# AvishaiBarnoy/membrane_solver

Measured on AMD Instinct MI355X. Metric: minimizer steps/sec (energy+grad+CG) on 2M-facet icosphere, higher is better.
Workload: dtype f64

## Files before the change

### include/membrane_hip.h

```cpp
#ifndef MEMBRANE_HIP_H
#define MEMBRANE_HIP_H

#include <stddef.h>
#include <stdint.h>

#ifdef __cplusplus
extern "C" {
#endif

#define MS_OK 0
#define MS_ERR_INVALID (-1)
#define MS_ERR_HIP (-2)
#define MS_ERR_TILE_CAPACITY (-3)
#define MS_ERR_STATE (-4)
#define MS_ERR_NOMEM (-5)

#define MS_MOD_SURFACE 1u
#define MS_MOD_BENDING 2u
#define MS_MOD_VOLUME_PENALTY 4u
#define MS_CON_VOLUME 8u
#define MS_TRACK_VOLUME 16u
#define MS_MOD_TILT 32u
#define MS_MOD_BENDING_TILT 64u
#define MS_MOD_TILT_SMOOTH 128u
// ... 275 lines not shown
                  double tol, ms_step_result *out);
int64_t ms_shard_exchange_count(const ms_ctx *ctx);
int ms_shard_chain_stats(const ms_ctx *ctx, int64_t stats[8]);
int ms_shard_comm_ranks(ms_ctx *ctx);
int ms_shard_peer_memory_kind(const ms_ctx *ctx);

size_t ms_state_bytes(const ms_ctx *ctx);
int ms_rebind_state(ms_ctx *ctx, void *device_base, size_t bytes);

int ms_device_buffer(ms_ctx *ctx, int buffer, void **dev_ptr, size_t *bytes);
int ms_shard_info(ms_ctx *ctx, int64_t *nvp, int64_t *row0, int64_t *row1,
                  int64_t *rows_per_shard);
int ms_tile_stats(ms_ctx *ctx, int64_t *n_tiles, int64_t *facet_instances,
                  int64_t *max_halo, int64_t *lds_bytes_energy,
                  int64_t *lds_bytes_gradient);

#define MS_PROF_KINDS 13
int ms_profile_enable(ms_ctx *ctx, int on);
int ms_profile_read(ms_ctx *ctx, double total_ms[MS_PROF_KINDS],
                    int64_t launches[MS_PROF_KINDS]);

int ms_queue_stats(ms_ctx *ctx, int64_t stats[8]);
int ms_direction_stats(ms_ctx *ctx, int64_t *skipped, int64_t *materialized);
int ms_exec_stats(ms_ctx *ctx, int64_t stats[4]);
int ms_resident_stats(ms_ctx *ctx, int64_t stats[4]);

#define MS_PIN_STAGE_FIXED 0
#define MS_PIN_STAGE_PLANE_GROUP 1
#define MS_PIN_STAGE_CIRCLE_GROUP 2
#define MS_PIN_OP_PLANE 0
// ... 44 lines not shown
```

### membrane_solver_amd/_lib.py

```python

from __future__ import annotations

import ctypes
import os
import subprocess

_PKG = os.path.dirname(os.path.abspath(__file__))
LIB_PATH = os.environ.get("MEMBRANE_HIP_LIB") or os.path.join(_PKG, "libmembrane_hip.so")
_CSRC = os.path.join(_PKG, "csrc")

MS_OK = 0
MS_ERR = {-1: "MS_ERR_INVALID", -2: "MS_ERR_HIP", -3: "MS_ERR_TILE_CAPACITY",
          -4: "MS_ERR_STATE", -5: "MS_ERR_NOMEM"}

MS_MOD_SURFACE = 1
MS_MOD_BENDING = 2
MS_MOD_VOLUME_PENALTY = 4
MS_CON_VOLUME = 8
MS_TRACK_VOLUME = 16
MS_MOD_TILT = 32
MS_MOD_BENDING_TILT = 64
MS_MOD_TILT_SMOOTH = 128
MS_MOD_TILT_IN, MS_MOD_TILT_OUT, MS_MOD_TILT_SMOOTH_IN, MS_MOD_TILT_SMOOTH_OUT = 256, 512, 1024, 2048
MS_MOD_BENDING_TILT_IN, MS_MOD_BENDING_TILT_OUT = 4096, 8192
# ... 167 lines not shown
    "ms_shard_set_allgather": (ctypes.c_int, [_P, ALLGATHER_FN, _P]),
    "ms_shard_step": (ctypes.c_int, [_P, ctypes.POINTER(ms_stepper_params), ctypes.c_double, ctypes.c_double,
                                     ctypes.POINTER(ms_step_result)]),
    "ms_shard_exchange_count": (ctypes.c_int64, [_P]),
    "ms_shard_chain_stats": (ctypes.c_int, [_P, _I64]),
    "ms_shard_comm_ranks": (ctypes.c_int, [_P]),
    "ms_shard_peer_memory_kind": (ctypes.c_int, [_P]),
    "ms_state_bytes": (ctypes.c_size_t, [_P]),
    "ms_rebind_state": (ctypes.c_int, [_P, _P, ctypes.c_size_t]),
    "ms_fetch_scalars": (ctypes.c_int, [_P, _D]),
    "ms_store_scalars": (ctypes.c_int, [_P, _D]),
    "ms_device_buffer": (ctypes.c_int, [_P, ctypes.c_int, ctypes.POINTER(_P),
                                        ctypes.POINTER(ctypes.c_size_t)]),
    "ms_shard_info": (ctypes.c_int, [_P, _I64, _I64, _I64, _I64]),
    "ms_tile_stats": (ctypes.c_int, [_P, _I64, _I64, _I64, _I64, _I64]),
    "ms_profile_enable": (ctypes.c_int, [_P, ctypes.c_int]),
    "ms_profile_read": (ctypes.c_int, [_P, _D, _I64]),
    "ms_queue_stats": (ctypes.c_int, [_P, _I64]),
    "ms_direction_stats": (ctypes.c_int, [_P, _I64, _I64]),
    "ms_exec_stats": (ctypes.c_int, [_P, _I64]),
    "ms_resident_stats": (ctypes.c_int, [_P, _I64]),
    "ms_set_pins": (ctypes.c_int, [_P, ctypes.c_int, _D, ctypes.c_int, _I32, _I32, _I32, _I32, _I32, ctypes.c_int,
                                   ctypes.c_int, _I32, _I32, _I32, ctypes.c_int, _I32, _I32, _I32]),
    "ms_enforce_pins": (ctypes.c_int, [_P]),
    "ms_pin_stats": (ctypes.c_int, [_P, _I64]),
    "ms_tsearch_stats": (ctypes.c_int, [_P, _I64]),
    "ms_exec_trace": (ctypes.c_int, [_P, ctypes.c_int, _D, ctypes.c_int, ctypes.POINTER(ctypes.c_int)]),
    "ms_shard_peer_export": (ctypes.c_int, [_P, _P]),
    "ms_shard_peer_open": (ctypes.c_int, [_P, _P]),
    "ms_shard_peer_local": (ctypes.c_int, [_P, ctypes.POINTER(_P), ctypes.POINTER(_P)]),
# ... 92 lines not shown
```

### membrane_solver_amd/csrc/ms_api_context.inc

```
extern "C" {

const char* ms_version(void) { return "membrane_hip 0.1 (gfx950)"; }

int ms_device_count(void) {
  int n = 0;
  hipError_t e = hipGetDeviceCount(&n);
  if (e != hipSuccess) {
    g_last_error = std::string("hipGetDeviceCount: ") + hipGetErrorString(e);
    return MS_ERR_HIP;
  }
  return n;
}

const char* ms_last_error(const ms_ctx* ctx) {
  return ctx ? ctx->err.c_str() : g_last_error.c_str();
}

int ms_create(ms_ctx** out, int device, int nv, int nf, const double* positions,
              const int32_t* tri, const uint8_t* fixed, const uint8_t* boundary,
              const uint8_t* body_facets, int tile_vertices, int shard_rank, int shard_count) {
  if (!out) return fail(nullptr, MS_ERR_INVALID, "ms_create: out is NULL");
  *out = nullptr;
  if (shard_count < 1 || shard_rank < 0 || shard_rank >= shard_count)
    return fail(nullptr, MS_ERR_INVALID, "ms_create: bad shard_rank/shard_count");
// ... 43 lines not shown
  CREATE_HIP(hipSetDevice(device));
  CREATE_HIP(hipStreamCreateWithFlags(&c->stream, hipStreamNonBlocking));
  c->own_stream = true;
  CREATE_CHK(upload(c, &c->d_perm, t.perm));
  CREATE_CHK(upload(c, &c->d_tile_facet_off, t.tile_facet_off));
  CREATE_CHK(upload(c, &c->d_tile_facets, t.tile_facets));
  if (t.own + t.max_halo <= 1024) {
    std::vector<uint32_t> packed(t.tile_facets.size());
    for (size_t i = 0; i < packed.size(); ++i) {
      const TileFacet& f = t.tile_facets[i];
      packed[i] = (uint32_t)f.l0 | ((uint32_t)f.l1 << 10) | ((uint32_t)f.l2 << 20) | ((uint32_t)(f.flags & 3u) << 30);
    }
    CREATE_CHK(upload(c, &c->d_tile_facets32, packed));
  }
  CREATE_CHK(upload(c, &c->d_tile_halo_off, t.tile_halo_off));
  CREATE_CHK(upload(c, &c->d_halo_ids, t.halo_ids));
  CREATE_CHK(upload(c, &c->d_tile_ent_off, t.tile_ent_off));
  CREATE_CHK(upload(c, &c->d_tile_voff, t.tile_voff));
  CREATE_CHK(upload(c, &c->d_vent, t.vent));
  {
    std::vector<double> ones(t.tile_facets.size(), 1.0);
    CREATE_CHK(upload(c, &c->d_tf_gamma, ones));
  }
  {
    std::vector<uint8_t> fl((size_t)t.nvp, VF_FIXED);
    for (int i = 0; i < nv; ++i) {
      const int e = t.perm[i];
      uint8_t f = 0;
      if (fixed && fixed[e]) f |= VF_FIXED;
      if (boundary && boundary[e]) {
// ... 128 lines not shown
            g_host_timing.n, g_host_timing.sum_gap / g_host_timing.n, g_host_timing.max_gap,
            g_host_timing.sum_launch / g_host_timing.n);
    g_host_timing.n = 0;
    g_host_timing.sum_gap = g_host_timing.sum_launch = g_host_timing.max_gap = 0.0;
  }
  if (!c) return;
  (void)hipSetDevice(c->device);
  if (c->exec_on) {
    (void)c->exec.flush();
    exec_detach(&c->exec);
    c->exec_on = false;
  }
  if (c->stream) (void)hipStreamSynchronize(c->stream);
  if (!c->own_state) c->state = nullptr;
  void* ptrs[] = {c->d_perm, c->d_tile_facet_off, c->d_tile_facets, c->d_tile_facets32, c->d_tf_gamma, c->d_volgrad_cache,
                  c->d_tile_halo_off, c->d_halo_ids, c->d_tile_ent_off, c->d_tile_voff, c->d_vent,
                  c->d_vflags, c->d_kappa, c->d_c0, c->tf[0].tilts, c->tf[0].grad, c->tf[0].trial, c->d_bt_vert, c->d_tn, c->tf[0].dir, c->tf[0].minv,
                  c->tf[1].tilts, c->tf[1].grad, c->tf[1].trial, c->tf[1].dir, c->tf[1].minv,
                  c->tf[2].tilts, c->tf[2].grad, c->tf[2].trial, c->tf[2].dir, c->tf[2].minv,
                  c->tf[1].kappa, c->tf[1].c0, c->tf[1].bt_vert, c->tf[2].kappa, c->tf[2].c0, c->tf[2].bt_vert,
                  c->tf[1].disk, c->tf[1].diff, c->tf[2].disk, c->tf[2].diff, c->tf[0].va, c->tf[1].va, c->tf[2].va,
                  c->state, c->d_partials, c->d_scal, c->d_stage, c->d_bnd_rows, c->d_bnd_off,
                  c->d_halo_rows, c->d_scal_all, c->d_pins, c->d_line, c->d_edgepen};
  for (void* p : ptrs)
    if (p) (void)hipFree(p);
  for (auto* prof : {c->line_prof, c->edgepen_prof})
    for (int w = 0; w < 2; ++w)
      for (auto& ev : prof[w]) {
        (void)hipEventDestroy(ev.first);
        (void)hipEventDestroy(ev.second);
      }
// ... 331 lines not shown
```

### membrane_solver_amd/csrc/ms_api_ctx.inc

```
struct StageCtl {
  const uint32_t* cur_gate = nullptr;
  uint32_t cur_gate_want = 0;
  bool cur_gate_fold_only = false;
  bool cur_check_ran = false;
  uint32_t* cur_dec = nullptr;
  double cur_rhs[MS_MAX_TRIALS] = {0};
  const double* cur_rhs_dev = nullptr;
  uint32_t cur_extra_mask = 0;
  int cur_go_kind = 0;
  uint32_t* cur_go = nullptr;
  double cur_go_val[6] = {0};
  int cur_parity = 0;
  int pair_on = 0;
  bool pair_lean = false;
  double pair_alpha[MS_MAX_TRIALS] = {0};
  double* pair_scal2 = nullptr;
  bool multi_any_slot = false;
  bool defer_dir = false;
  bool energy_tilt_only = false;
  bool proj_at_x_in_normals = false;
};
struct CarryState {
  bool dir_implicit = false;
  bool dir_unwritten = false;
// ... 16 lines not shown
  Tiling til;
  int shard_rank = 0, shard_count = 1;
  int tile0 = 0, tile1 = 0;
  int cap = 0;
  int32_t* d_perm = nullptr;
  int32_t* d_tile_facet_off = nullptr;
  TileFacet* d_tile_facets = nullptr;
  uint32_t* d_tile_facets32 = nullptr;
  double* d_tf_gamma = nullptr;
  double* d_volgrad_cache = nullptr;
  double volgrad_cache_norm2 = 0.0;
  bool volgrad_cache_valid = false;
  bool gamma_uniform = true, kc_uniform = true;
  double gamma_const = 1.0, kappa_const = 0.0, c0_const = 0.0;
  int32_t* d_tile_halo_off = nullptr;
  int32_t* d_halo_ids = nullptr;
  int32_t* d_tile_ent_off = nullptr;
  uint16_t* d_tile_voff = nullptr;
  uint16_t* d_vent = nullptr;
  uint8_t* d_vflags = nullptr;
  double* d_kappa = nullptr;
  double* d_c0 = nullptr;
  struct TiltField {
    double* tilts = nullptr;
    double* trial = nullptr;
    double* grad = nullptr;
    double* dir = nullptr;
    double* minv = nullptr;
    double k_tilt = 0.0;
    int consistent = 0;
// ... 230 lines not shown
```

### membrane_solver_amd/csrc/ms_api_misc.inc

```
size_t ms_state_bytes(const ms_ctx* c) {
  if (!c) return 0;
  return sizeof(double) * (8 * 3 * (size_t)c->til.nvp + 2 * (size_t)c->til.nvp);
}

int ms_rebind_state(ms_ctx* c, void* device_base, size_t bytes) {
  if (!c || !device_base) return fail(c, MS_ERR_INVALID, "ms_rebind_state: NULL argument");
  const size_t need = ms_state_bytes(c);
  if (bytes < need) return fail(c, MS_ERR_INVALID, "ms_rebind_state: buffer smaller than ms_state_bytes");
  HIPCHK(c, hipStreamSynchronize(S(c)));
  HIPCHK(c, hipMemcpy(device_base, c->state, need, hipMemcpyDeviceToDevice));
  double* nb = static_cast<double*>(device_base);
  for (int b = 0; b <= MS_BUF_FA; ++b) c->buf[b] = nb + (c->buf[b] - c->state);
  c->carry.last_g = nb + (c->carry.last_g - c->state);
  if (c->own_state) HIPCHK(c, hipFree(c->state));
  c->state = nb;
  c->own_state = false;
  return MS_OK;
}

int ms_fetch_scalars(ms_ctx* c, double* out) {
  if (!c || !out) return MS_ERR_INVALID;
  int rc = fetch(c);
  if (rc) return rc;
  memcpy(out, c->h_scal, sizeof(double) * MS_NSCAL);
// ... 34 lines not shown
  return MS_OK;
}

int ms_tile_stats(ms_ctx* c, int64_t* n_tiles, int64_t* facet_instances, int64_t* max_halo,
                  int64_t* lds_bytes_energy, int64_t* lds_bytes_gradient) {
  if (!c) return MS_ERR_INVALID;
  const Tiling& t = c->til;
  const bool bend = (c->params.modules & MS_MOD_BENDING) != 0;
  if (n_tiles) *n_tiles = t.n_tiles;
  if (facet_instances) *facet_instances = (int64_t)t.tile_facets.size();
  if (max_halo) *max_halo = t.max_halo;
  if (lds_bytes_energy) *lds_bytes_energy = (int64_t)energy_lds_bytes(t.T, c->cap, t.max_ent, bend, false, c->has_boundary, !c->deterministic);
  if (lds_bytes_gradient)
    *lds_bytes_gradient = (int64_t)gradient_lds_bytes(t.T, c->cap, t.max_ent, bend,
                                                      (c->params.modules & MS_CON_VOLUME) != 0, !c->deterministic);
  return MS_OK;
}

int ms_queue_stats(ms_ctx* c, int64_t stats[8]) {
  if (!c || !stats) return MS_ERR_INVALID;
  for (int k = 0; k < 8; ++k) stats[k] = 0;
  stats[0] = c->q_rounds;
  stats[1] = c->q_multi;
  stats[2] = c->q_wasted;
  stats[3] = c->q_side_accepts;
  stats[4] = c->queue_mismatches;
  stats[5] = c->q_ahead;
  stats[6] = c->q_adopted;
  stats[7] = c->q_dropped;
  return MS_OK;
// ... 341 lines not shown
```

### membrane_solver_amd/csrc/ms_api_phases.inc

```
namespace {

inline hipStream_t S(ms_ctx* c) {
  if (c->exec_on) (void)c->exec.flush();
  return c->stream;
}
int pin_grad_run(ms_ctx* c, bool volrow);
int line_energy_run(ms_ctx* c, bool use_dir, double alpha);
int line_grad_run(ms_ctx* c, double* g, bool volrow);
int edgepen_energy_run(ms_ctx* c, bool use_dir, double alpha);
int edgepen_grad_run(ms_ctx* c, double* g, bool volrow);
inline int exec_flush(ms_ctx* c) {
  if (!c->exec_on) return MS_OK;
  const hipError_t e = c->exec.flush();
  if (e == hipSuccess) return MS_OK;
  c->err = std::string("k_exec launch: ") + hipGetErrorString(e);
  return MS_ERR_HIP;
}

inline int zero_doubles(ms_ctx* c, double* p, size_t bytes) {
  if (c->exec_on) {
    ExecMemsetArgs a;
    a.p = p;
    a.n = (int64_t)(bytes / sizeof(double));
    const hipError_t e = c->exec.push(CK_MEMSET, 0, 0, 0, 1, 0, 0, &a, sizeof(a));
// ... 32 lines not shown
  m.T = c->til.T;
  m.own = c->til.own;
  m.n_tiles = c->til.n_tiles;
  m.has_boundary = c->has_boundary ? 1 : 0;
  m.tile_facet_off = c->d_tile_facet_off;
  m.tile_facets = c->d_tile_facets;
  m.tile_facets32 = c->d_tile_facets32;
  m.no_fast = c->no_fast ? 1 : 0;
  m.tf_gamma = c->d_tf_gamma;
  m.gamma_uniform = c->gamma_uniform ? 1 : 0;
  m.gamma_const = c->gamma_const;
  m.kc_uniform = c->kc_uniform ? 1 : 0;
  m.kappa_const = c->kappa_const;
  m.c0_const = c->c0_const;
  m.tile_halo_off = c->d_tile_halo_off;
  m.halo_ids = c->d_halo_ids;
  m.tile_ent_off = c->d_tile_ent_off;
  m.tile_voff = c->d_tile_voff;
  m.vent = c->d_vent;
  m.vflags = c->d_vflags;
  m.kappa = c->d_kappa;
  m.c0 = c->d_c0;
  return m;
}

struct HostTiming {
  bool on = getenv("MS_HOST_TIMING") != nullptr && atoi(getenv("MS_HOST_TIMING")) != 0;
  double t_fetch = 0.0;
  bool armed = false;
  double sum_gap = 0.0, sum_launch = 0.0, max_gap = 0.0;
// ... 984 lines not shown
```

### membrane_solver_amd/csrc/ms_exec.inc

```

typedef const __attribute__((address_space(4))) unsigned char* exec_kptr;
#define MS_EXEC_FN

__device__ __forceinline__ exec_kptr exec_uniform_ptr(exec_kptr p) {
  const unsigned long long v = (unsigned long long)p;
  const unsigned int lo = (unsigned int)__builtin_amdgcn_readfirstlane((int)(unsigned int)v);
  const unsigned int hi = (unsigned int)__builtin_amdgcn_readfirstlane((int)(unsigned int)(v >> 32));
  return (exec_kptr)(((unsigned long long)hi << 32) | lo);
}
template <int SKIP, typename A>
__device__ __forceinline__ void exec_load(A& dst, exec_kptr src) {
  static_assert(SKIP % 8 == 0 && sizeof(A) % 8 == 0, "8-byte granules");
  typedef const __attribute__((address_space(4))) unsigned long long* q8;
  unsigned long long w[(sizeof(A) - SKIP) / 8];
#pragma unroll
  for (int i = 0; i < (int)((sizeof(A) - SKIP) / 8); ++i) w[i] = ((q8)src)[i];
  __builtin_memcpy(reinterpret_cast<char*>(&dst) + SKIP, w, sizeof(A) - SKIP);
}
__device__ __forceinline__ int exec_uniform(int v) { return __builtin_amdgcn_readfirstlane(v); }

static_assert(offsetof(EnergyArgs, m) == 0 && offsetof(GradientArgs, m) == 0 && offsetof(TiltArgs, m) == 0 &&
                  offsetof(BtArgs, m) == 0 && offsetof(TsArgs, m) == 0,
              "the tile kernels' argument structs start with their DeviceMesh");
static_assert(sizeof(DeviceMesh) % 8 == 0, "DeviceMesh is a whole number of 8-byte granules");
// ... 263 lines not shown
      exec_run_one(base, off, lds);
      off += (int)h.bytes;
    }
  }
}

namespace {
constexpr int EXEC_SLOTS = 32;
std::atomic<ExecRecorder*> g_exec_slots[EXEC_SLOTS];
std::atomic<int> g_exec_count{0};
bool same_mesh(const DeviceMesh& a, const DeviceMesh& b) {
  return a.nv == b.nv && a.T == b.T && a.n_tiles == b.n_tiles && a.own == b.own && a.has_boundary == b.has_boundary &&
         a.tile_facet_off == b.tile_facet_off && a.tile_facets == b.tile_facets && a.tile_facets32 == b.tile_facets32 &&
         a.no_fast == b.no_fast && a.tf_gamma == b.tf_gamma && a.gamma_uniform == b.gamma_uniform &&
         a.kc_uniform == b.kc_uniform && a.gamma_const == b.gamma_const && a.kappa_const == b.kappa_const &&
         a.c0_const == b.c0_const && a.tile_halo_off == b.tile_halo_off && a.halo_ids == b.halo_ids &&
         a.tile_ent_off == b.tile_ent_off && a.tile_voff == b.tile_voff && a.vent == b.vent && a.vflags == b.vflags &&
         a.kappa == b.kappa && a.c0 == b.c0;
}
}

ExecRecorder* exec_find(hipStream_t s) {
  if (g_exec_count.load(std::memory_order_acquire) == 0) return nullptr;
  for (int i = 0; i < EXEC_SLOTS; ++i) {
    ExecRecorder* r = g_exec_slots[i].load(std::memory_order_acquire);
    if (r != nullptr && r->stream == s) return r;
  }
  return nullptr;
}
void exec_attach(ExecRecorder* r) {
  for (int i = 0; i < EXEC_SLOTS; ++i) {
// ... 155 lines not shown
```

### membrane_solver_amd/csrc/ms_internal.h

```cpp
#pragma once

#include <hip/hip_runtime.h>

#include <cstdint>
#include <cstdlib>
#include <string>
#include <vector>

#include "membrane_hip.h"

namespace ms {

inline const char* variant_env(const char* name) {
#ifdef MS_VARIANT_ENV
  return getenv(name);
#else
  (void)name;
  return nullptr;
#endif
}

struct TileFacet {
  uint16_t l0, l1, l2;
  uint16_t flags;
// ... 25 lines not shown
constexpr uint8_t VF_TILT_FIXED_IN = 8;
constexpr uint8_t VF_TILT_FIXED_OUT = 16;

struct Tiling {
  int nv = 0, nf = 0, T = 256;
  int own = 256;
  int n_tiles = 0;
  int n_tiles_padded = 0;
  int tiles_per_shard = 0;
  int64_t nvp = 0;
  std::vector<int32_t> perm;
  std::vector<int32_t> iperm;
  std::vector<int32_t> tile_facet_off;
  std::vector<TileFacet> tile_facets;
  std::vector<int32_t> tile_facet_ext;
  std::vector<int32_t> tile_halo_off;
  std::vector<int32_t> halo_ids;
  std::vector<int32_t> tile_ent_off;
  std::vector<uint16_t> tile_voff;
  std::vector<uint16_t> vent;
  int max_ent = 0;
  int max_halo = 0;
  int max_tile_facets = 0;
  int64_t dropped_facets = 0;
};

int build_tiling(int nv, int nf, const double* positions, const int32_t* tri,
                 const uint8_t* body_facets, int T, int shard_count, Tiling& out,
                 std::string& err);

struct DeviceMesh {
  int nv, T, n_tiles;
  int own;
  int has_boundary;
  const int32_t* tile_facet_off;
  const TileFacet* tile_facets;
  const uint32_t* tile_facets32;
  int no_fast;
  const double* tf_gamma;
  int gamma_uniform, kc_uniform;
  double gamma_const, kappa_const, c0_const;
  const int32_t* tile_halo_off;
  const int32_t* halo_ids;
  const int32_t* tile_ent_off;
  const uint16_t* tile_voff;
  const uint16_t* vent;
  const uint8_t* vflags;
  const double* kappa;
  const double* c0;
};
// ... 622 lines not shown
```

### membrane_solver_amd/csrc/ms_kernels.hip

```cpp
#include <hip/hip_runtime.h>
#include <atomic>
#include <cstddef>
#include <cstdio>
#include <cstdlib>
#include <cstring>
#include <ctime>
#include <mutex>
#include <type_traits>

#include "ms_internal.h"

#ifndef MS_RSQRT_NORM
#define MS_RSQRT_NORM 1
#endif

namespace ms {

struct V3 {
  double x, y, z;
};
__device__ __forceinline__ V3 mk(double x, double y, double z) { return V3{x, y, z}; }
__device__ __forceinline__ V3 operator-(V3 a, V3 b) { return mk(a.x - b.x, a.y - b.y, a.z - b.z); }
__device__ __forceinline__ V3 operator+(V3 a, V3 b) { return mk(a.x + b.x, a.y + b.y, a.z + b.z); }
__device__ __forceinline__ V3 operator-(V3 a) { return mk(-a.x, -a.y, -a.z); }
// ... 262 lines not shown
__device__ __forceinline__ TileFacet facet_unpack(const FacetRec<PACKED>& r) {
  if constexpr (PACKED) {
    TileFacet f;
    f.l0 = (uint16_t)(r.v & 1023u);
    f.l1 = (uint16_t)((r.v >> 10) & 1023u);
    f.l2 = (uint16_t)((r.v >> 20) & 1023u);
    f.flags = (uint16_t)(r.v >> 30);
    return f;
  } else {
    return r.v;
  }
}

struct TileCtx {
  int tile, v_lo, n_owned, h0, nh, f0, f1, e0, n_ent;
};
__device__ __forceinline__ TileCtx tile_ctx(const DeviceMesh& m, int tile) {
  TileCtx t;
  t.tile = tile;
  t.v_lo = tile * m.own;
  t.n_owned = min(m.own, m.nv - t.v_lo);
  t.h0 = m.tile_halo_off[tile];
  t.nh = m.tile_halo_off[tile + 1] - t.h0;
  t.f0 = m.tile_facet_off[tile];
  t.f1 = m.tile_facet_off[tile + 1];
#ifdef MS_ABL_CLAMP
  t.f1 = min(t.f1, t.f0 + MS_ABL_CLAMP);
#endif
  t.e0 = m.tile_ent_off[tile];
  t.n_ent = m.tile_ent_off[tile + 1] - t.e0;
  return t;
}

#ifndef MS_WPE_ENERGY
#define MS_WPE_ENERGY
#endif
#ifndef MS_WPE_GRADIENT
#define MS_WPE_GRADIENT
#endif
#ifndef MS_KA_SLOTS
#define MS_KA_SLOTS 5
#endif
#ifndef MS_LEAN_SLOTS
#define MS_LEAN_SLOTS 5
#endif
constexpr int CSR_REGS = 12;
struct CsrStage {
  uint16_t vo0, vo1;
  uint16_t e[CSR_REGS];
};
__device__ __forceinline__ void csr_issue(CsrStage& r, const DeviceMesh& m, const TileCtx& t, int T,
                                          int tid) {
  const uint16_t* gv = m.tile_voff + (size_t)t.tile * (T + 1);
  r.vo0 = gv[tid];
  r.vo1 = gv[tid + 1];
  const uint16_t* ge = m.vent + t.e0;
#pragma unroll
  for (int k = 0; k < CSR_REGS; ++k) {
    const int j = tid + k * T;
// ... 74 lines not shown
  (void)blk;
  MS_STAMP(0);
  MS_STAMP_ID();
  const TileCtx t = tile_ctx(a.m, my_tile);
  const int tid = threadIdx.x;
  const bool have_d = a.d != nullptr;

  constexpr bool PACKED = TT == 256;
  FacetRec<PACKED> tf_nx = facet_null<PACKED>();
  double gam_nx = 0.0;
  if (t.f0 + tid < t.f1) {
    tf_nx = facet_load<PACKED>(a.m, (size_t)(t.f0 + tid));
    gam_nx = a.m.gamma_uniform ? a.m.gamma_const : a.m.tf_gamma[t.f0 + tid];
  }

  double kappa_v = 0.0, c0_v = 0.0;
  if (BEND && tid < t.n_owned) {
    kappa_v = a.m.kc_uniform ? a.m.kappa_const : a.m.kappa[t.v_lo + tid];
    c0_v = a.m.kc_uniform ? a.m.c0_const : a.m.c0[t.v_lo + tid];
  }

  uint8_t own_fl = 0;
  int cur = 0, end = 0;
  {
    const bool own = tid < t.n_owned;
    const int v_own = t.v_lo + tid;
    const bool has_h = tid < t.nh;
    int hv = 0;
    if (has_h) hv = a.m.halo_ids[t.h0 + tid];
    double xo0 = 0, xo1 = 0, xo2 = 0, dd0 = 0, dd1 = 0, dd2 = 0;
    uint8_t fl = 0;
    if (own) {
      const size_t g = 3 * (size_t)v_own;
      fl = a.m.vflags[v_own];
      xo0 = a.x[g];
      xo1 = a.x[g + 1];
      xo2 = a.x[g + 2];
      if (have_d) {
        dd0 = a.d[g];
        dd1 = a.d[g + 1];
        dd2 = a.d[g + 2];
      }
    }
    CsrStage cs;
    if (BEND && !ATOMIC) csr_issue(cs, a.m, t, T, tid);
    if (BEND && ATOMIC) {
      for (int j = tid; j < 5 * T; j += T) stg[j] = 0.0;
    }
    own_fl = fl;
    double h0 = 0, h1 = 0, h2 = 0, e0 = 0, e1 = 0, e2 = 0;
    uint8_t hfl = 0;
    if (has_h) {
      const size_t g = 3 * (size_t)hv;
      hfl = a.m.vflags[hv];
      h0 = a.x[g];
      h1 = a.x[g + 1];
      h2 = a.x[g + 2];
      if (have_d) {
        e0 = a.d[g];
        e1 = a.d[g + 1];
        e2 = a.d[g + 2];
      }
    }
    if (own) {
      const size_t g = 3 * (size_t)v_own;
      const bool mv = have_d && !(fl & VF_FIXED);
      const double x0 = mv ? axpy1(xo0, a.alpha, dd0) : xo0;
      const double x1 = mv ? axpy1(xo1, a.alpha, dd1) : xo1;
      const double x2 = mv ? axpy1(xo2, a.alpha, dd2) : xo2;
      if (stage_flags) lfl[tid] = fl;
      lds_put3(px, tid, x0, x1, x2);
      if (GUARD) lds_put3(ox, tid, xo0, xo1, xo2);
      if (a.xt) {
        a.xt[g] = x0;
        a.xt[g + 1] = x1;
        a.xt[g + 2] = x2;
      }
    }
    if (BEND && !ATOMIC) {
      csr_commit(cs, a.m, t, T, tid, vent);
      cur = cs.vo0;
      end = cs.vo1;
    }
    if (has_h) {
      const int s = t.n_owned + tid;
      const bool mv = have_d && !(hfl & VF_FIXED);
      if (stage_flags) lfl[s] = hfl;
      lds_put3(px, s, mv ? axpy1(h0, a.alpha, e0) : h0, mv ? axpy1(h1, a.alpha, e1) : h1, mv ? axpy1(h2, a.alpha, e2) : h2);
      if (GUARD) lds_put3(ox, s, h0, h1, h2);
    }
    for (int h = tid + T; h < t.nh; h += T) {
      const int v = a.m.halo_ids[t.h0 + h];
      const size_t g = 3 * (size_t)v;
      const uint8_t f2 = a.m.vflags[v];
      const double q0 = a.x[g], q1 = a.x[g + 1], q2 = a.x[g + 2];
      double r0 = 0, r1 = 0, r2 = 0;
      if (have_d) {
        r0 = a.d[g];
        r1 = a.d[g + 1];
        r2 = a.d[g + 2];
      }
      const int s = t.n_owned + h;
      const bool mv = have_d && !(f2 & VF_FIXED);
      if (stage_flags) lfl[s] = f2;
      lds_put3(px, s, mv ? axpy1(q0, a.alpha, r0) : q0, mv ? axpy1(q1, a.alpha, r1) : q1, mv ? axpy1(q2, a.alpha, r2) : q2);
// ... 1 lines not shown
    }
  }
  __syncthreads();
  MS_STAMP(1);

  double e_surf = 0.0, vol = 0.0, min_e2 = 1.0e300, guard = 0.0;
  const bool want_surf = a.modules & MS_MOD_SURFACE;
  const bool want_vol = a.modules & (MS_MOD_VOLUME_PENALTY | MS_CON_VOLUME | MS_TRACK_VOLUME);
  constexpr bool want_area = AREA;
  double area = 0.0;
  double aKx = 0, aKy = 0, aKz = 0, aAv = 0, aAe = 0;
  if (!(BEND && tid < t.n_owned)) cur = end = 0;
  const int ent_begin = cur;

  for (int c0 = t.f0; c0 < t.f1; c0 += T) {
    const int p = c0 + tid;
    const TileFacet tf = facet_unpack<PACKED>(tf_nx);
    const double gam = gam_nx;
    if (p + T < t.f1) {
      tf_nx = facet_load<PACKED>(a.m, (size_t)(p + T));
      gam_nx = a.m.gamma_uniform ? a.m.gamma_const : a.m.tf_gamma[p + T];
    }
    double va0 = 0, va1 = 0, va2 = 0, ve0 = 0, ve1 = 0, ve2 = 0;
    if (p < t.f1) {
      const bool owner = tf.flags & TF_OWNER;
      if (BEND || owner) {
        const V3 v0 = lds_row3(px, tf.l0), v1 = lds_row3(px, tf.l1), v2 = lds_row3(px, tf.l2);
        const V3 e0 = v2 - v1, e1 = v0 - v2, e2 = v1 - v0;
        const double l0 = dot(e0, e0), l1 = dot(e1, e1), l2 = dot(e2, e2);
        const V3 n = cross(e2, -e1);
// ... 102 lines not shown
        s[0 * T] = va0; s[1 * T] = va1; s[2 * T] = va2;
        s[3 * T] = ve0; s[4 * T] = ve1; s[5 * T] = ve2;
      }
      __syncthreads();
      for (int q = cur0; q < cur; ++q) {
        const int ent = vent[q];
        const double* s = stg + ((ent >> 2) - lo) + (ent & 3) * T;
        aAv += s[0];
        aAe += s[3 * T];
      }
      __syncthreads();
    }
  }

  if (BEND && ATOMIC) {
    __syncthreads();
    MS_STAMP(2);
    if (tid < t.n_owned) {
      aKx = stg[tid];
      aKy = stg[T + tid];
      aKz = stg[2 * T + tid];
      aAv = stg[3 * T + tid];
      aAe = aAv + stg[4 * T + tid];
    }
    __syncthreads();
  }
  double e_bend = 0.0;
  if (BEND && tid < t.n_owned) {
    const int v = t.v_lo + tid;
    const V3 K = mk(aKx, aKy, aKz);
    const double kappa = kappa_v, c0 = c0_v;
    const bool interior = !(own_fl & VF_BOUNDARY);
    const double safe = fmax(aAv, 1.0e-12);
    double k_mag, inv_k_mag;
    norm_and_inverse(dot(K, K), k_mag, inv_k_mag);
    const double inv_safe = 1.0 / safe;
    double H = k_mag * (0.5 * inv_safe);
    const bool signed_h = a.bt_normals != nullptr;
    V3 nh = mk(0, 0, 0);
    if (signed_h) {
      nh = mk(a.bt_normals[3 * (size_t)v], a.bt_normals[3 * (size_t)v + 1], a.bt_normals[3 * (size_t)v + 2]);
      H = dot(K, nh) * (0.5 * inv_safe);
    }
    const double ratio = safe > 1.0e-15 ? aAe * inv_safe : 0.0;
    double scale_K, fe, fv;
    if (a.bt_vert) {
// ... 2654 lines not shown
```

### membrane_solver_amd/csrc/ms_tiles.cpp

```cpp
#include <algorithm>
#include <cstdlib>
#include <cmath>
#include <cstring>
#include <numeric>

#include "ms_internal.h"

namespace ms {

namespace {

inline uint64_t hilbert3(uint32_t x, uint32_t y, uint32_t z, int bits) {
  uint32_t X[3] = {x, y, z};
  const uint32_t M = 1u << (bits - 1);
  for (uint32_t Q = M; Q > 1; Q >>= 1) {
    uint32_t P = Q - 1;
    for (int i = 0; i < 3; ++i) {
      if (X[i] & Q) {
        X[0] ^= P;
      } else {
        uint32_t t = (X[0] ^ X[i]) & P;
        X[0] ^= t;
        X[i] ^= t;
      }
// ... 157 lines not shown
    for (int j = 0; j < n; ++j) {
      size_t p = (size_t)cursor[tl[j]]++;
      inst_v[3 * p] = iv[0];
      inst_v[3 * p + 1] = iv[1];
      inst_v[3 * p + 2] = iv[2];
      uint16_t fl = 0;
      if (tl[j] == owner_tile) fl |= TF_OWNER;
      if (!body_facets || body_facets[f]) fl |= TF_BODY;
      out.tile_facets[p].flags = fl;
      out.tile_facet_ext[p] = f;
    }
  }

  out.tile_halo_off.assign(out.n_tiles + 1, 0);
  out.tile_ent_off.assign(out.n_tiles + 1, 0);
  out.tile_voff.assign((size_t)out.n_tiles * (T + 1), 0);
  std::vector<int32_t> halo_tmp;
  std::vector<int32_t> vcnt(T + 1);
  const char* env_order = variant_env("MS_FACET_ORDER");
  const int order_mode = env_order ? atoi(env_order) : 2;
  const char* env_stride = getenv("MS_FACET_STRIDE");
  const int stride_mode = env_stride ? atoi(env_stride) : 1;
  std::vector<TileFacet> tf_tmp;
  std::vector<int32_t> ext_tmp;
  std::vector<int32_t> order;
  std::vector<uint8_t> taken;
  for (int t = 0; t < out.n_tiles; ++t) {
    const int v_lo = t * R;
    const int v_hi = std::min(nv, v_lo + R);
    const size_t b = (size_t)out.tile_facet_off[t], e = (size_t)out.tile_facet_off[t + 1];
// ... 15 lines not shown
      uint16_t loc[3];
      for (int k = 0; k < 3; ++k) {
        int v = inst_v[3 * p + k];
        if (v >= v_lo && v < v_hi) {
          loc[k] = (uint16_t)(v - v_lo);
        } else {
          auto it = std::lower_bound(halo_tmp.begin(), halo_tmp.end(), v);
          loc[k] = (uint16_t)(n_owned + (int)(it - halo_tmp.begin()));
        }
      }
      out.tile_facets[p].l0 = loc[0];
      out.tile_facets[p].l1 = loc[1];
      out.tile_facets[p].l2 = loc[2];
    }

    if (n >= 128 && order_mode != 0) {
      tf_tmp.assign(out.tile_facets.begin() + b, out.tile_facets.begin() + e);
      ext_tmp.assign(out.tile_facet_ext.begin() + b, out.tile_facet_ext.begin() + e);
      order.clear();
      order.reserve(n);
      size_t S = std::max<size_t>(stride_mode > 1 ? (size_t)stride_mode : 7, (n + 63) / 64);
      while (std::gcd(S, n) != 1) ++S;
      std::vector<int32_t>& cand = order;
      for (size_t i = 0; i < n; ++i) cand.push_back((int32_t)((i * S) % n));
      if (order_mode >= 2) {
        std::vector<int32_t> seq(cand);
        taken.assign(n, 0);
        order.clear();
        size_t first_free = 0;
        while (order.size() < n) {
          uint32_t m32[3] = {0, 0, 0};
          const size_t group_end = std::min(n, order.size() + 32);
          for (int half = 0; half < 2 && order.size() < group_end; ++half) {
            uint32_t m16[3] = {0, 0, 0};
            const size_t half_end = std::min(group_end, order.size() + 16);
            while (order.size() < half_end) {
              size_t best = n;
              int best_cost = 99, seen = 0;
              for (size_t q = first_free; q < n && seen < 192; ++q) {
                if (taken[q]) continue;
                ++seen;
                const TileFacet& f = tf_tmp[seq[q]];
                const uint32_t r[3] = {f.l0, f.l1, f.l2};
                int cost = 0;
                for (int k = 0; k < 3; ++k)
                  cost += (int)((m32[k] >> (r[k] & 31)) & 1u) + (int)((m16[k] >> (r[k] & 15)) & 1u);
                if (cost < best_cost) {
                  best_cost = cost;
                  best = q;
                  if (cost == 0) break;
                }
              }
              if (best == n) break;
              const TileFacet& f = tf_tmp[seq[best]];
              const uint32_t r[3] = {f.l0, f.l1, f.l2};
              for (int k = 0; k < 3; ++k) {
                m32[k] |= 1u << (r[k] & 31);
                m16[k] |= 1u << (r[k] & 15);
              }
              taken[best] = 1;
              order.push_back(seq[best]);
              while (first_free < n && taken[first_free]) ++first_free;
            }
            while (first_free < n && taken[first_free]) ++first_free;
          }
        }
      }
      for (size_t i = 0; i < n; ++i) {
        out.tile_facets[b + i] = tf_tmp[order[i]];
        out.tile_facet_ext[b + i] = ext_tmp[order[i]];
      }
    }

    {
      if (e - b > 16383u) {
        err = "ms_create: a tile lists more than 16383 facets (vertex valence too high)";
        return MS_ERR_TILE_CAPACITY;
      }
      std::fill(vcnt.begin(), vcnt.end(), 0);
// ... 37 lines not shown
```

### membrane_solver_amd/device.py

```python

from __future__ import annotations

import ctypes
from dataclasses import dataclass

import numpy as np

from . import _lib as L


def _f64(a, shape=None, name="array"):
    a = np.ascontiguousarray(a, dtype=np.float64)
    if shape is not None and a.shape != tuple(shape):
        raise ValueError(f"{name} must have shape {tuple(shape)}, got {a.shape}")
    return a


def _pd(a):
    return None if a is None else a.ctypes.data_as(L._D)


def _pu8(a):
    return None if a is None else a.ctypes.data_as(L._U8)

# ... 588 lines not shown
            kind, mi, cnt, tot = int(rows[k, 0]), int(rows[k, 1]), int(rows[k, 2]), float(rows[k, 3])
            out.append({"kind": self.EXEC_KINDS.get(kind, str(kind)), "mode": mi & 0xffff, "inst": mi >> 16, "count": cnt,
                        "total_us": tot, "avg_us": tot / max(cnt, 1)})
        return out

    def shard_info(self):
        v = [ctypes.c_int64(0) for _ in range(4)]
        self._chk(L.lib().ms_shard_info(self._h, *[ctypes.byref(x) for x in v]), "ms_shard_info")
        return {"nvp": v[0].value, "row0": v[1].value, "row1": v[2].value, "rows_per_shard": v[3].value}

    def tile_stats(self):
        v = [ctypes.c_int64(0) for _ in range(5)]
        self._chk(L.lib().ms_tile_stats(self._h, *[ctypes.byref(x) for x in v]), "ms_tile_stats")
        return {"n_tiles": v[0].value, "facet_instances": v[1].value, "max_halo": v[2].value,
                "lds_bytes_energy": v[3].value, "lds_bytes_gradient": v[4].value}
```

Baseline: 19300.

## Sort tile facets interior-first and defer halo LDS commit past first facet chunk

Tile facets are reordered so facets whose three vertices are all owned come first, and the per-tile interior count is stored and uploaded to the device. In the atomic bending gradient kernel with 256-thread tiles, the halo vertex loads are kept in registers and written to LDS only after the first facet chunk, when that chunk touches no halo vertices. This lets the global halo gathers overlap with interior facet compute. Per-vertex kappa/c0 loads are also deferred. The cost is extra register pressure, an extra barrier, and a bank-conflict ordering heuristic now applied separately within each class.

```diff
diff --git a/include/membrane_hip.h b/include/membrane_hip.h
--- a/include/membrane_hip.h
+++ b/include/membrane_hip.h
@@ -313,6 +313,8 @@
 int ms_tile_stats(ms_ctx *ctx, int64_t *n_tiles, int64_t *facet_instances,
                   int64_t *max_halo, int64_t *lds_bytes_energy,
                   int64_t *lds_bytes_gradient);
+int ms_tile_interior(ms_ctx *ctx, int32_t *facets, int32_t *interior,
+                     int32_t *halo_rows);
 
 #define MS_PROF_KINDS 13
 int ms_profile_enable(ms_ctx *ctx, int on);
diff --git a/membrane_solver_amd/_lib.py b/membrane_solver_amd/_lib.py
--- a/membrane_solver_amd/_lib.py
+++ b/membrane_solver_amd/_lib.py
@@ -205,6 +205,7 @@
                                         ctypes.POINTER(ctypes.c_size_t)]),
     "ms_shard_info": (ctypes.c_int, [_P, _I64, _I64, _I64, _I64]),
     "ms_tile_stats": (ctypes.c_int, [_P, _I64, _I64, _I64, _I64, _I64]),
+    "ms_tile_interior": (ctypes.c_int, [_P, _I32, _I32, _I32]),
     "ms_profile_enable": (ctypes.c_int, [_P, ctypes.c_int]),
     "ms_profile_read": (ctypes.c_int, [_P, _D, _I64]),
     "ms_queue_stats": (ctypes.c_int, [_P, _I64]),
diff --git a/membrane_solver_amd/csrc/ms_api_context.inc b/membrane_solver_amd/csrc/ms_api_context.inc
--- a/membrane_solver_amd/csrc/ms_api_context.inc
+++ b/membrane_solver_amd/csrc/ms_api_context.inc
@@ -81,6 +81,7 @@
     CREATE_CHK(upload(c, &c->d_tile_facets32, packed));
   }
   CREATE_CHK(upload(c, &c->d_tile_halo_off, t.tile_halo_off));
+  CREATE_CHK(upload(c, &c->d_tile_fint, t.tile_fint));
   CREATE_CHK(upload(c, &c->d_halo_ids, t.halo_ids));
   CREATE_CHK(upload(c, &c->d_tile_ent_off, t.tile_ent_off));
   CREATE_CHK(upload(c, &c->d_tile_voff, t.tile_voff));
@@ -239,7 +240,7 @@
   if (c->stream) (void)hipStreamSynchronize(c->stream);
   if (!c->own_state) c->state = nullptr;
   void* ptrs[] = {c->d_perm, c->d_tile_facet_off, c->d_tile_facets, c->d_tile_facets32, c->d_tf_gamma, c->d_volgrad_cache,
-                  c->d_tile_halo_off, c->d_halo_ids, c->d_tile_ent_off, c->d_tile_voff, c->d_vent,
+                  c->d_tile_halo_off, c->d_tile_fint, c->d_halo_ids, c->d_tile_ent_off, c->d_tile_voff, c->d_vent,
                   c->d_vflags, c->d_kappa, c->d_c0, c->tf[0].tilts, c->tf[0].grad, c->tf[0].trial, c->d_bt_vert, c->d_tn, c->tf[0].dir, c->tf[0].minv,
                   c->tf[1].tilts, c->tf[1].grad, c->tf[1].trial, c->tf[1].dir, c->tf[1].minv,
                   c->tf[2].tilts, c->tf[2].grad, c->tf[2].trial, c->tf[2].dir, c->tf[2].minv,
diff --git a/membrane_solver_amd/csrc/ms_api_ctx.inc b/membrane_solver_amd/csrc/ms_api_ctx.inc
--- a/membrane_solver_amd/csrc/ms_api_ctx.inc
+++ b/membrane_solver_amd/csrc/ms_api_ctx.inc
@@ -54,6 +54,7 @@
   bool gamma_uniform = true, kc_uniform = true;
   double gamma_const = 1.0, kappa_const = 0.0, c0_const = 0.0;
   int32_t* d_tile_halo_off = nullptr;
+  int32_t* d_tile_fint = nullptr;
   int32_t* d_halo_ids = nullptr;
   int32_t* d_tile_ent_off = nullptr;
   uint16_t* d_tile_voff = nullptr;
diff --git a/membrane_solver_amd/csrc/ms_api_misc.inc b/membrane_solver_amd/csrc/ms_api_misc.inc
--- a/membrane_solver_amd/csrc/ms_api_misc.inc
+++ b/membrane_solver_amd/csrc/ms_api_misc.inc
@@ -72,6 +72,17 @@
   if (lds_bytes_gradient)
     *lds_bytes_gradient = (int64_t)gradient_lds_bytes(t.T, c->cap, t.max_ent, bend,
                                                       (c->params.modules & MS_CON_VOLUME) != 0, !c->deterministic);
+  return MS_OK;
+}
+
+int ms_tile_interior(ms_ctx* c, int32_t* facets, int32_t* interior, int32_t* halo_rows) {
+  if (!c) return MS_ERR_INVALID;
+  const Tiling& t = c->til;
+  for (int tile = 0; tile < t.n_tiles; ++tile) {
+    if (facets) facets[tile] = t.tile_facet_off[tile + 1] - t.tile_facet_off[tile];
+    if (interior) interior[tile] = t.tile_fint[tile];
+    if (halo_rows) halo_rows[tile] = t.tile_halo_off[tile + 1] - t.tile_halo_off[tile];
+  }
   return MS_OK;
 }
 
diff --git a/membrane_solver_amd/csrc/ms_api_phases.inc b/membrane_solver_amd/csrc/ms_api_phases.inc
--- a/membrane_solver_amd/csrc/ms_api_phases.inc
+++ b/membrane_solver_amd/csrc/ms_api_phases.inc
@@ -70,6 +70,7 @@
   m.kappa_const = c->kappa_const;
   m.c0_const = c->c0_const;
   m.tile_halo_off = c->d_tile_halo_off;
+  m.tile_fint = c->d_tile_fint;
   m.halo_ids = c->d_halo_ids;
   m.tile_ent_off = c->d_tile_ent_off;
   m.tile_voff = c->d_tile_voff;
diff --git a/membrane_solver_amd/csrc/ms_exec.inc b/membrane_solver_amd/csrc/ms_exec.inc
--- a/membrane_solver_amd/csrc/ms_exec.inc
+++ b/membrane_solver_amd/csrc/ms_exec.inc
@@ -301,7 +301,7 @@
          a.tile_facet_off == b.tile_facet_off && a.tile_facets == b.tile_facets && a.tile_facets32 == b.tile_facets32 &&
          a.no_fast == b.no_fast && a.tf_gamma == b.tf_gamma && a.gamma_uniform == b.gamma_uniform &&
          a.kc_uniform == b.kc_uniform && a.gamma_const == b.gamma_const && a.kappa_const == b.kappa_const &&
-         a.c0_const == b.c0_const && a.tile_halo_off == b.tile_halo_off && a.halo_ids == b.halo_ids &&
+         a.c0_const == b.c0_const && a.tile_halo_off == b.tile_halo_off && a.tile_fint == b.tile_fint && a.halo_ids == b.halo_ids &&
          a.tile_ent_off == b.tile_ent_off && a.tile_voff == b.tile_voff && a.vent == b.vent && a.vflags == b.vflags &&
          a.kappa == b.kappa && a.c0 == b.c0;
 }
diff --git a/membrane_solver_amd/csrc/ms_internal.h b/membrane_solver_amd/csrc/ms_internal.h
--- a/membrane_solver_amd/csrc/ms_internal.h
+++ b/membrane_solver_amd/csrc/ms_internal.h
@@ -63,6 +63,7 @@
   std::vector<int32_t> tile_facet_off;
   std::vector<TileFacet> tile_facets;
   std::vector<int32_t> tile_facet_ext;
+  std::vector<int32_t> tile_fint;
   std::vector<int32_t> tile_halo_off;
   std::vector<int32_t> halo_ids;
   std::vector<int32_t> tile_ent_off;
@@ -83,6 +84,7 @@
   int own;
   int has_boundary;
   const int32_t* tile_facet_off;
+  const int32_t* tile_fint;
   const TileFacet* tile_facets;
   const uint32_t* tile_facets32;
   int no_fast;
diff --git a/membrane_solver_amd/csrc/ms_kernels.hip b/membrane_solver_amd/csrc/ms_kernels.hip
--- a/membrane_solver_amd/csrc/ms_kernels.hip
+++ b/membrane_solver_amd/csrc/ms_kernels.hip
@@ -300,6 +300,7 @@
 
 struct TileCtx {
   int tile, v_lo, n_owned, h0, nh, f0, f1, e0, n_ent;
+  int fint;
 };
 __device__ __forceinline__ TileCtx tile_ctx(const DeviceMesh& m, int tile) {
   TileCtx t;
@@ -313,6 +314,7 @@
 #ifdef MS_ABL_CLAMP
   t.f1 = min(t.f1, t.f0 + MS_ABL_CLAMP);
 #endif
+  t.fint = m.tile_fint[tile];
   t.e0 = m.tile_ent_off[tile];
   t.n_ent = m.tile_ent_off[tile + 1] - t.e0;
   return t;
@@ -329,6 +331,9 @@
 #endif
 #ifndef MS_LEAN_SLOTS
 #define MS_LEAN_SLOTS 5
+#endif
+#ifndef MS_HALO_OVERLAP
+#define MS_HALO_OVERLAP 1
 #endif
 constexpr int CSR_REGS = 12;
 struct CsrStage {
@@ -433,14 +438,27 @@
     gam_nx = a.m.gamma_uniform ? a.m.gamma_const : a.m.tf_gamma[t.f0 + tid];
   }
 
+  constexpr bool OVERLAP = MS_HALO_OVERLAP && ATOMIC && BEND && !GUARD && !AREA && TT == 256;
   double kappa_v = 0.0, c0_v = 0.0;
-  if (BEND && tid < t.n_owned) {
+  if (BEND && !OVERLAP && tid < t.n_owned) {
     kappa_v = a.m.kc_uniform ? a.m.kappa_const : a.m.kappa[t.v_lo + tid];
     c0_v = a.m.kc_uniform ? a.m.c0_const : a.m.c0[t.v_lo + tid];
   }
 
   uint8_t own_fl = 0;
   int cur = 0, end = 0;
+  bool halo_pending = false;
+  double hp0 = 0, hp1 = 0, hp2 = 0, he0 = 0, he1 = 0, he2 = 0;
+  uint8_t hpf = 0;
+  auto commit_halo = [&](double h0, double h1, double h2, double e0, double e1, double e2, uint8_t hfl) {
+    if (tid < t.nh) {
+      const int s = t.n_owned + tid;
+      const bool mv = have_d && !(hfl & VF_FIXED);
+      if (stage_flags) lfl[s] = hfl;
+      lds_put3(px, s, mv ? axpy1(h0, a.alpha, e0) : h0, mv ? axpy1(h1, a.alpha, e1) : h1, mv ? axpy1(h2, a.alpha, e2) : h2);
+      if (GUARD) lds_put3(ox, s, h0, h1, h2);
+    }
+  };
   {
     const bool own = tid < t.n_owned;
     const int v_own = t.v_lo + tid;
@@ -467,11 +485,17 @@
       for (int j = tid; j < 5 * T; j += T) stg[j] = 0.0;
     }
     own_fl = fl;
+    const bool mv_own = have_d && !(fl & VF_FIXED);
+    const double x0 = mv_own ? axpy1(xo0, a.alpha, dd0) : xo0;
+    const double x1 = mv_own ? axpy1(xo1, a.alpha, dd1) : xo1;
+    const double x2 = mv_own ? axpy1(xo2, a.alpha, dd2) : xo2;
+    if (OVERLAP) asm volatile("" ::"v"(x0), "v"(x1), "v"(x2), "v"((int)fl), "v"(hv));
     double h0 = 0, h1 = 0, h2 = 0, e0 = 0, e1 = 0, e2 = 0;
     uint8_t hfl = 0;
     if (has_h) {
-      const size_t g = 3 * (size_t)hv;
-      hfl = a.m.vflags[hv];
+      const size_t hvi = OVERLAP ? (size_t)(uint32_t)hv : (size_t)hv;
+      const size_t g = 3 * hvi;
+      hfl = a.m.vflags[hvi];
       h0 = a.x[g];
       h1 = a.x[g + 1];
       h2 = a.x[g + 2];
@@ -483,10 +507,6 @@
     }
     if (own) {
       const size_t g = 3 * (size_t)v_own;
-      const bool mv = have_d && !(fl & VF_FIXED);
-      const double x0 = mv ? axpy1(xo0, a.alpha, dd0) : xo0;
-      const double x1 = mv ? axpy1(xo1, a.alpha, dd1) : xo1;
-      const double x2 = mv ? axpy1(xo2, a.alpha, dd2) : xo2;
       if (stage_flags) lfl[tid] = fl;
       lds_put3(px, tid, x0, x1, x2);
       if (GUARD) lds_put3(ox, tid, xo0, xo1, xo2);
@@ -501,13 +521,12 @@
       cur = cs.vo0;
       end = cs.vo1;
     }
-    if (has_h) {
-      const int s = t.n_owned + tid;
-      const bool mv = have_d && !(hfl & VF_FIXED);
-      if (stage_flags) lfl[s] = hfl;
-      lds_put3(px, s, mv ? axpy1(h0, a.alpha, e0) : h0, mv ? axpy1(h1, a.alpha, e1) : h1, mv ? axpy1(h2, a.alpha, e2) : h2);
-      if (GUARD) lds_put3(ox, s, h0, h1, h2);
-    }
+    if (OVERLAP) {
+      halo_pending = t.fint >= T && t.nh <= T;
+      hp0 = h0; hp1 = h1; hp2 = h2; he0 = e0; he1 = e1; he2 = e2;
+      hpf = hfl;
+    }
+    if (!halo_pending) commit_halo(h0, h1, h2, e0, e1, e2, hfl);
     for (int h = tid + T; h < t.nh; h += T) {
       const int v = a.m.halo_ids[t.h0 + h];
       const size_t g = 3 * (size_t)v;
@@ -539,6 +558,11 @@
   const int ent_begin = cur;
 
   for (int c0 = t.f0; c0 < t.f1; c0 += T) {
+    if (OVERLAP && halo_pending && c0 != t.f0) {
+      commit_halo(hp0, hp1, hp2, he0, he1, he2, hpf);
+      halo_pending = false;
+      __syncthreads();
+    }
     const int p = c0 + tid;
     const TileFacet tf = facet_unpack<PACKED>(tf_nx);
     const double gam = gam_nx;
@@ -671,6 +695,11 @@
   }
 
   if (BEND && ATOMIC) {
+    if (OVERLAP && halo_pending) commit_halo(hp0, hp1, hp2, he0, he1, he2, hpf);
+    if (OVERLAP && !a.m.kc_uniform && tid < t.n_owned) {
+      kappa_v = a.m.kappa[t.v_lo + tid];
+      c0_v = a.m.c0[t.v_lo + tid];
+    }
     __syncthreads();
     MS_STAMP(2);
     if (tid < t.n_owned) {
@@ -686,7 +715,8 @@
   if (BEND && tid < t.n_owned) {
     const int v = t.v_lo + tid;
     const V3 K = mk(aKx, aKy, aKz);
-    const double kappa = kappa_v, c0 = c0_v;
+    const double kappa = (OVERLAP && a.m.kc_uniform) ? a.m.kappa_const : kappa_v;
+    const double c0 = (OVERLAP && a.m.kc_uniform) ? a.m.c0_const : c0_v;
     const bool interior = !(own_fl & VF_BOUNDARY);
     const double safe = fmax(aAv, 1.0e-12);
     double k_mag, inv_k_mag;
diff --git a/membrane_solver_amd/csrc/ms_tiles.cpp b/membrane_solver_amd/csrc/ms_tiles.cpp
--- a/membrane_solver_amd/csrc/ms_tiles.cpp
+++ b/membrane_solver_amd/csrc/ms_tiles.cpp
@@ -195,6 +195,7 @@
 
   out.tile_halo_off.assign(out.n_tiles + 1, 0);
   out.tile_ent_off.assign(out.n_tiles + 1, 0);
+  out.tile_fint.assign(out.n_tiles, 0);
   out.tile_voff.assign((size_t)out.n_tiles * (T + 1), 0);
   std::vector<int32_t> halo_tmp;
   std::vector<int32_t> vcnt(T + 1);
@@ -240,55 +241,83 @@
       out.tile_facets[p].l2 = loc[2];
     }
 
-    if (n >= 128 && order_mode != 0) {
+    {
       tf_tmp.assign(out.tile_facets.begin() + b, out.tile_facets.begin() + e);
       ext_tmp.assign(out.tile_facet_ext.begin() + b, out.tile_facet_ext.begin() + e);
+      auto interior = [&](const TileFacet& f) { return f.l0 < n_owned && f.l1 < n_owned && f.l2 < n_owned; };
       order.clear();
       order.reserve(n);
-      size_t S = std::max<size_t>(stride_mode > 1 ? (size_t)stride_mode : 7, (n + 63) / 64);
-      while (std::gcd(S, n) != 1) ++S;
-      std::vector<int32_t>& cand = order;
-      for (size_t i = 0; i < n; ++i) cand.push_back((int32_t)((i * S) % n));
-      if (order_mode >= 2) {
-        std::vector<int32_t> seq(cand);
-        taken.assign(n, 0);
+      for (size_t i = 0; i < n; ++i)
+        if (interior(tf_tmp[i])) order.push_back((int32_t)i);
+      const size_t n_int = order.size();
+      for (size_t i = 0; i < n; ++i)
+        if (!interior(tf_tmp[i])) order.push_back((int32_t)i);
+      out.tile_fint[t] = (int32_t)n_int;
+      if (n >= 128 && order_mode != 0) {
+        const std::vector<int32_t> walk(order);
         order.clear();
-        size_t first_free = 0;
-        while (order.size() < n) {
-          uint32_t m32[3] = {0, 0, 0};
-          const size_t group_end = std::min(n, order.size() + 32);
-          for (int half = 0; half < 2 && order.size() < group_end; ++half) {
-            uint32_t m16[3] = {0, 0, 0};
-            const size_t half_end = std::min(group_end, order.size() + 16);
-            while (order.size() < half_end) {
-              size_t best = n;
-              int best_cost = 99, seen = 0;
-              for (size_t q = first_free; q < n && seen < 192; ++q) {
-                if (taken[q]) continue;
-                ++seen;
-                const TileFacet& f = tf_tmp[seq[q]];
+        for (int cls = 0; cls < 2; ++cls) {
+          const size_t c_lo = cls == 0 ? 0 : n_int, m = cls == 0 ? n_int : n - n_int;
+          if (m == 0) continue;
+          size_t S = std::max<size_t>(stride_mode > 1 ? (size_t)stride_mode : 7, (m + 63) / 64);
+          while (std::gcd(S, m) != 1) ++S;
+          std::vector<int32_t> seq(m);
+          for (size_t i = 0; i < m; ++i) seq[i] = walk[c_lo + (i * S) % m];
+          if (order_mode < 2) {
+            order.insert(order.end(), seq.begin(), seq.end());
+            continue;
+          }
+          taken.assign(m, 0);
+          const size_t done0 = order.size();
+          size_t first_free = 0;
+          while (order.size() - done0 < m) {
+            uint32_t m32[3] = {0, 0, 0};
+            const size_t group_lo = order.size() & ~(size_t)31;
+            const size_t group_end = std::min(done0 + m, group_lo + 32);
+            auto mark = [&](uint32_t* mask, uint32_t mod, size_t lo) {
+              for (size_t i = lo; i < order.size(); ++i) {
+                const TileFacet& f = tf_tmp[order[i]];
+                mask[0] |= 1u << (f.l0 & mod);
+                mask[1] |= 1u << (f.l1 & mod);
+                mask[2] |= 1u << (f.l2 & mod);
+              }
+            };
+            mark(m32, 31, group_lo);
+            while (order.size() < group_end) {
+              uint32_t m16[3] = {0, 0, 0};
+              const size_t half_lo = order.size() & ~(size_t)15;
+              const size_t half_end = std::min(group_end, half_lo + 16);
+              mark(m16, 15, half_lo);
+              while (order.size() < half_end) {
+                size_t best = m;
+                int best_cost = 99, seen = 0;
+                for (size_t q = first_free; q < m && seen < 192; ++q) {
+                  if (taken[q]) continue;
+                  ++seen;
+                  const TileFacet& f = tf_tmp[seq[q]];
+                  const uint32_t r[3] = {f.l0, f.l1, f.l2};
+                  int cost = 0;
+                  for (int k = 0; k < 3; ++k)
+                    cost += (int)((m32[k] >> (r[k] & 31)) & 1u) + (int)((m16[k] >> (r[k] & 15)) & 1u);
+                  if (cost < best_cost) {
+                    best_cost = cost;
+                    best = q;
+                    if (cost == 0) break;
+                  }
+                }
+                if (best == m) break;
+                const TileFacet& f = tf_tmp[seq[best]];
                 const uint32_t r[3] = {f.l0, f.l1, f.l2};
-                int cost = 0;
-                for (int k = 0; k < 3; ++k)
-                  cost += (int)((m32[k] >> (r[k] & 31)) & 1u) + (int)((m16[k] >> (r[k] & 15)) & 1u);
-                if (cost < best_cost) {
-                  best_cost = cost;
-                  best = q;
-                  if (cost == 0) break;
+                for (int k = 0; k < 3; ++k) {
+                  m32[k] |= 1u << (r[k] & 31);
+                  m16[k] |= 1u << (r[k] & 15);
                 }
+                taken[best] = 1;
+                order.push_back(seq[best]);
+                while (first_free < m && taken[first_free]) ++first_free;
               }
-              if (best == n) break;
-              const TileFacet& f = tf_tmp[seq[best]];
-              const uint32_t r[3] = {f.l0, f.l1, f.l2};
-              for (int k = 0; k < 3; ++k) {
-                m32[k] |= 1u << (r[k] & 31);
-                m16[k] |= 1u << (r[k] & 15);
-              }
-              taken[best] = 1;
-              order.push_back(seq[best]);
-              while (first_free < n && taken[first_free]) ++first_free;
+              while (first_free < m && taken[first_free]) ++first_free;
             }
-            while (first_free < n && taken[first_free]) ++first_free;
           }
         }
       }
diff --git a/membrane_solver_amd/device.py b/membrane_solver_amd/device.py
--- a/membrane_solver_amd/device.py
+++ b/membrane_solver_amd/device.py
@@ -626,3 +626,9 @@
         self._chk(L.lib().ms_tile_stats(self._h, *[ctypes.byref(x) for x in v]), "ms_tile_stats")
         return {"n_tiles": v[0].value, "facet_instances": v[1].value, "max_halo": v[2].value,
                 "lds_bytes_energy": v[3].value, "lds_bytes_gradient": v[4].value}
+
+    def tile_interior(self):
+        n = self.tile_stats()["n_tiles"]
+        v = [np.zeros(n, np.int32) for _ in range(3)]
+        self._chk(L.lib().ms_tile_interior(self._h, *[x.ctypes.data_as(L._I32) for x in v]), "ms_tile_interior")
+        return {"facets": v[0], "interior": v[1], "halo_rows": v[2]}
```

Result: slower. 19040 (-1.3%).
